# moriglia/qam-reconciliation

Hardware: AMD Instinct MI355X
Metric: decoded frames/sec @ N=64800, 50 BP iters; achieved HBM GB/s vs roofline (higher is better)
Workload: dtype f64; 1 GPU; dvbs2_4pam; code=DVB-S2-rate-1/2-profile IRA N=64800, V=64800, C=32400, E=226799, batch_per_gpu=4096, global_batch=4096, bps=2, fused_demap=False, parallelism=dp1, hip_graph=False, backend=none, arithmetic=strict (glibc exp/log restated: outputs bit-identical to the reference)

## Files before the change

### qam-reconciliation_amd/csrc/decoder.hip

```cpp
#include <atomic>
#include <functional>

#include "debug_check.hpp"
#include "glibc_math.hpp"
#include "qamr_internal.hpp"
#include "strict_pack.hpp"
#include "host_build.hpp"

namespace qr {

enum CheckMode { kFirst = 0, kNormal = 1, kParityOnly = 2 };

enum DebugSite {
    kDbgLaneFrame = 1,
    kDbgNarrowFrame = 2,
    kDbgNarrowNode = 3,
    kDbgRepackList = 4,
    kDbgRepackSlot = 5,
    kDbgRepackFid = 6,
    kDbgCompact = 7,
    kDbgResPost = 8,
    kDbgResMsg = 9,
    kDbgFewCheck = 17,
    kDbgFewPost = 18,
// ... 79 lines not shown
    double *post;
    const uint8_t *active;
    int ld, f_off;
    Geom g;
    unsigned nbx;
    const int32_t *alist, *acount;
    unsigned nby;
    int gs;
    int boost;
    int32_t *finite;
    double fin_bound;
    int fin_B;
    const int32_t *sel;
    const double *lappr_w[2];
    double *post_w;
    const double *c2v_alt;
    int transit;
};

enum RangeSelField { kSelOn = 0, kSelW = 1, kSelRepacks = 2, kSelArrive = 3, kSelBuf = 4, kSelTransit = 5, kSelInts = 6 };

__device__ __forceinline__ void select_range(CheckArgs &a) {
    if (a.sel && sld(a.sel + kSelOn)) {
        const int b = sld(a.sel + kSelBuf);
        a.post = a.post_w;
        a.synd = b ? a.synd_w[1] : a.synd_w[0];
        double *const c0 = a.c2v, *const c1 = a.c2v_alt;
        a.c2v = b ? c1 : c0;
        a.transit = sld(a.sel + kSelTransit);
        a.c2v_rd = a.transit ? (b ? c0 : c1) : a.c2v;
    }
}
__device__ __forceinline__ void select_range(VarArgs &a) {
    if (a.sel && sld(a.sel + kSelOn)) {
        const int b = sld(a.sel + kSelBuf);
        a.lappr = b ? a.lappr_w[1] : a.lappr_w[0];
        a.post = a.post_w;
        a.transit = sld(a.sel + kSelTransit);
        if (a.transit ? !b : b) a.c2v = a.c2v_alt;
    }
}

__device__ __forceinline__ bool frames_block_live(const int32_t *acount, unsigned by, int lft) {
    return !acount || (int)(by << lft) < *acount;
}
__device__ __forceinline__ int lane_frame(const int32_t *alist, const int32_t *acount, int f_off, int p, bool &live) {
    live = true;
    if (!alist) return f_off + p;
    const int cnt = *acount;
    live = p < cnt;
    const int f = alist[f_off + (live ? p : cnt - 1)];
    QR_DCHECK(f >= f_off + (live ? p : cnt - 1), kDbgLaneFrame, f, f_off + p);
    return f;
}


template <int D, int MODE, bool NT, bool TRANSIT = false>
struct CheckIn {
    double p[D], c[D];
    int base;
    uint8_t sb;
    __device__ __forceinline__ void load(const CheckArgs &a, int64_t ci, int f) {
        const int ld = a.ld;
        const uint32_t b8 = (uint32_t)f * 8u;
        const int cc = sld(a.checks + ci);
        base = sld(a.chk_ptr + cc);
        sb = *at_byte(row_ptr(a.synd, cc, ld), (uint32_t)f);
#pragma unroll
        for (int i = 0; i < D; ++i) p[i] = ld_row<false>(row_ptr(a.post, sld(a.chk_var + base + i), ld), b8, ld);
    }
    __device__ __forceinline__ void load_c(const CheckArgs &a, int fc) {
        if (MODE != kNormal) return;
        const uint32_t b8 = (uint32_t)fc * 8u;
        const double *c2v = TRANSIT ? a.c2v_rd : a.c2v;
#pragma unroll
        for (int i = 0; i < D; ++i) c[i] = ld_row<NT>(row_ptr(c2v, sld(a.chk_edge + base + i), a.ld), b8, a.ld);
    }
};

__device__ __forceinline__ uint32_t sign_mask(uint8_t sb) { return sb ? 0x80000000u : 0u; }
__device__ __forceinline__ double apply_sign(double x, uint32_t smask) { return g_make(g_hi(x) ^ smask, g_lo(x)); }

constexpr int kPackMaxDeg = 10;
constexpr int kPackLdsDoubles = 4 * kPackWaveDoubles;
template <int D>
constexpr bool kPacked = D <= kPackMaxDeg;

template <int D, bool NT, bool FIN = false>
__device__ __forceinline__ void check_exact(const CheckArgs &a, const double (&m)[D], int base, uint8_t sb, uint32_t b8,
                                            const GlibcTablesBP &tab, const GlibcK &K, double *hb = nullptr,
                                            bool live = true) {
    const int ld = a.ld;
    const double s = sb ? -1.0 : 1.0;
    if constexpr (kPacked<D>) {
        double out[D];
        double *wb = hb + (threadIdx.x >> 6) * kPackWaveDoubles;
        check_strict_packed<D, FIN ? kClampFinite : kClampFull>(m, out, wb, tab, K);
        const uint32_t smask = sign_mask(sb);
#pragma unroll
        for (int i = 0; i < D; ++i)
            if (live) st_row<NT>(row_ptr(a.c2v, sld(a.chk_edge + base + i), ld), b8, ld, apply_sign(out[i], smask));
        return;
    }
    double F[D - 1];
    F[0] = m[0];
#pragma unroll
    for (int i = 1; i < D - 1; ++i) F[i] = box_plus_strict(F[i - 1], m[i], tab, K);
    if (live) st_row<NT>(row_ptr(a.c2v, sld(a.chk_edge + base + D - 1), ld), b8, ld, s * F[D - 2]);
    double Bn = m[D - 1];
#pragma unroll
    for (int i = D - 2; i > 0; --i) {
        const double o = s * box_plus_strict(F[i - 1], Bn, tab, K);
        if (live) st_row<NT>(row_ptr(a.c2v, sld(a.chk_edge + base + i), ld), b8, ld, o);
        Bn = box_plus_strict(Bn, m[i], tab, K);
    }
    if (live) st_row<NT>(row_ptr(a.c2v, sld(a.chk_edge + base), ld), b8, ld, s * Bn);
}

template <int D, int MODE, bool NT, bool FIN = false, bool TRANSIT = false>
__device__ __forceinline__ void check_block(const CheckArgs &a, unsigned bx, unsigned by, int per,
                                            const GlibcTablesBP &tab, double *hb) {
    const int ft = 1 << a.g.lft;
    const int nsub = 256 >> a.g.lft;
    bool live;
    const int lp = (int)(by << a.g.lft) + (threadIdx.x & (ft - 1));
    const int fl = lane_frame(a.alist, a.acount, a.f_off, lp, live);
    const int f = TRANSIT ? a.f_off + lp : fl;
    const int sub = __builtin_amdgcn_readfirstlane(threadIdx.x >> a.g.lft);
    const bool act = live && a.active[f] != 0;
    if (!wave_any(act)) return;
    int64_t ci = (int64_t)bx * per * nsub + sub;
    if (ci >= a.n_checks) return;
    uint32_t bad = 0;
    const auto K = GlibcK::pinned();
    constexpr bool kPrefetch = !kPacked<D>;
    CheckIn<D, MODE, NT, TRANSIT> nx;
    nx.load(a, ci, f);
    for (int j = 0; j < per; ++j) {
        nx.load_c(a, TRANSIT ? fl : f);
        uint32_t par = nx.sb;
        double m[D];
#pragma unroll
        for (int i = 0; i < D; ++i) {
            const double p = nx.p[i];
            if (MODE != kFirst) par ^= (p < 0.0) ? 1u : 0u;
            if (MODE == kNormal) m[i] = p - nx.c[i];
            else m[i] = p;
        }
        struct { int base; uint8_t sb; } cur = {nx.base, nx.sb};
        const int64_t cn = ci + nsub;
        const bool more = (j + 1 < per) && cn < a.n_checks;
        if (kPrefetch && more) nx.load(a, cn, f);
        if (MODE != kFirst) bad |= (par == 1u) ? 1u : 0u;
        if (MODE != kParityOnly) {
            const uint32_t b8 = (uint32_t)f * 8u;
            check_exact<D, NT, FIN>(a, m, cur.base, cur.sb, b8, tab, K, hb, live);
        }
        if (!more) break;
        if (!kPrefetch) nx.load(a, cn, f);
        ci = cn;
    }
    if (MODE != kFirst && bad && act && live) a.unsat[f] = 1;
}

template <bool INIT, bool NT, bool TRANSIT = false>
__device__ __forceinline__ void var_block(const VarArgs &a, unsigned bx, unsigned by) {
    const int ft = 1 << a.g.lft;
    const int nsub = 256 >> a.g.lft;
    const int ld = a.ld;
    bool live;
    const int lp = (int)(by << a.g.lft) + (threadIdx.x & (ft - 1));
    const int fl = lane_frame(a.alist, a.acount, a.f_off, lp, live);
    const int f = TRANSIT ? a.f_off + lp : fl;
    const int fc = TRANSIT ? fl : f;
    const int sub = __builtin_amdgcn_readfirstlane(threadIdx.x >> a.g.lft);
    const bool act = a.active[f] != 0;
    if (!live || (!INIT && !act)) return;
    if (INIT && f >= a.fin_B) return;
    const int64_t v0 = (int64_t)bx * a.g.per * nsub + sub;
    bool big = false;
    for (int j = 0; j < a.g.per; ++j) {
        const int64_t v = v0 + (int64_t)j * nsub;
        if (v >= a.V) break;
        const int b = sld(a.var_ptr + v), e = sld(a.var_ptr + v + 1);
        double p = ld_msg<NT>(&a.lappr[(size_t)v * ld + f]);
        if (INIT) {
            big |= !(__builtin_fabs(p) < a.fin_bound);
            if (act && e > b) p = p + 0.0;
        } else {
            for (int k = b; k < e; ++k) p += ld_msg<NT>(&a.c2v[(size_t)sld(a.var_edge + k) * ld + fc]);
        }
        a.post[(size_t)v * ld + f] = p;
    }
    if (INIT && a.finite && big && f < a.fin_B) *a.finite = 0;
}

constexpr int kNarrowFrames = 16;
constexpr int kNarrowNodes = 256 / kNarrowFrames;
constexpr int kNarrowW = 64;

__device__ __forceinline__ bool range_narrow(const int32_t *sel, const int32_t *acount) {
    return sel && acount && sld(sel + kSelOn) && sld(sel + kSelW) <= kNarrowW && !sld(sel + kSelTransit);
}
__device__ __forceinline__ uint32_t narrow_tasks(int64_t n, const int32_t *acount, int &lg) {
    const int ngrp = (sld(acount) + kNarrowFrames - 1) / kNarrowFrames;
    lg = ngrp > 2 ? 2 : ngrp > 1 ? 1 : 0;
    return ngrp > 0 ? (uint32_t)((n + kNarrowNodes - 1) / kNarrowNodes) << lg : 0u;
}

template <int D>
__device__ __forceinline__ void check_narrow(const CheckArgs &a, uint32_t task, int lg, const GlibcTablesBP &tab,
                                             double *hb, const GlibcK &K) {
    bool live;
    const int grp = (int)(task & ((1u << lg) - 1u));
    const int f = lane_frame(a.alist, a.acount, a.f_off, grp * kNarrowFrames + (int)(threadIdx.x % kNarrowFrames), live);
    const bool act = live && a.active[f] != 0;
    if (!wave_any(act)) return;
    const int64_t ci = (int64_t)(task >> lg) * kNarrowNodes + threadIdx.x / kNarrowFrames;
    const bool valid = ci < a.n_checks;
    const int cc = a.checks[valid ? ci : a.n_checks - 1];
    int base = a.chk_ptr[cc];
    QR_DCHECK(f >= a.f_off && f < a.f_off + kNarrowW, kDbgNarrowFrame, f, a.f_off);
    QR_DCHECK(cc >= 0 && base >= 0 && a.chk_ptr[cc + 1] - base == D, kDbgNarrowNode, cc, base);
    const size_t ld = a.ld;
    const uint8_t sb = a.synd[(size_t)cc * ld + f];
    uint32_t par = sb;
    double m[D];
#pragma unroll
    for (int i = 0; i < D; ++i) {
        const double p = a.post[(size_t)a.chk_var[base + i] * ld + f];
        par ^= (p < 0.0) ? 1u : 0u;
        m[i] = p - a.c2v[(size_t)a.chk_edge[base + i] * ld + f];
    }
    double out[D];
    check_strict_packed<D, kClampFull>(m, out, hb + (threadIdx.x >> 6) * kPackWaveDoubles, tab, K);
    __asm__ volatile("" : "+v"(base));
    const double s = sb ? -1.0 : 1.0;
    if (valid && act) {
#pragma unroll
        for (int i = 0; i < D; ++i) a.c2v[(size_t)a.chk_edge[base + i] * ld + f] = s * out[i];
        if (par == 1u) a.unsat[f] = 1;
    }
}

template <int D>
__device__ __forceinline__ void check_narrow_sweep(const CheckArgs &a, GlibcTablesBP &tab, double *hb) {
    int lg;
    const uint32_t ntask = narrow_tasks(a.n_checks, a.acount, lg);
    const uint32_t nb = gridDim.x * gridDim.y, b = blockIdx.y * gridDim.x + blockIdx.x;
    if (b >= ntask) return;
    stage_glibc_tables(&tab, a.gglibc);
    const auto K = GlibcK::pinned();
    for (uint32_t t = b; t < ntask; t += nb) check_narrow<D>(a, t, lg, tab, hb, K);
}

__device__ __forceinline__ void var_narrow_sweep(const VarArgs &a) {
    int lg;
    const uint32_t ntask = narrow_tasks(a.V, a.acount, lg);
    const uint32_t nb = gridDim.x * gridDim.y;
    const size_t ld = a.ld;
    for (uint32_t t = blockIdx.y * gridDim.x + blockIdx.x; t < ntask; t += nb) {
        bool live;
        const int grp = (int)(t & ((1u << lg) - 1u));
        const int f = lane_frame(a.alist, a.acount, a.f_off, grp * kNarrowFrames + (int)(threadIdx.x % kNarrowFrames), live);
        const int64_t v = (int64_t)(t >> lg) * kNarrowNodes + threadIdx.x / kNarrowFrames;
        if (!live || v >= a.V || !a.active[f]) continue;
        QR_DCHECK(f >= a.f_off && f < a.f_off + kNarrowW, kDbgNarrowFrame, f, a.f_off);
        double p = a.lappr[(size_t)v * ld + f];
        const int b = a.var_ptr[v], e = a.var_ptr[v + 1];
        for (int k = b; k < e; ++k) p += a.c2v[(size_t)a.var_edge[k] * ld + f];
        a.post[(size_t)v * ld + f] = p;
    }
}

#if QR_EXPERIMENT_CLOCK
__device__ unsigned long long g_clk[3];
__device__ unsigned long long g_wgt[2 * kWgTimes];
#endif
template <int D, int MODE, bool NT>
__global__ void __launch_bounds__(256) __attribute__((amdgpu_waves_per_eu(1, 8))) k_check(CheckArgs a) {
    __shared__ GlibcTablesBP tab;
    __shared__ double hb[kPackLdsDoubles];
    select_range(a);
    if constexpr (MODE == kNormal && kPacked<D>) {
        if (range_narrow(a.sel, a.acount)) {
            check_narrow_sweep<D>(a, tab, hb);
            return;
        }
    }
    unsigned bx = blockIdx.x, by = blockIdx.y;
    int per = a.g.per;
    if (a.nmain) {
        if (bx < a.nmain) {
            by = 1 + bx / a.nbx;
            bx -= (by - 1) * a.nbx;
        } else {
            bx -= a.nmain;
            by = 0;
            per = a.per_t;
        }
    }
    if (!frames_block_live(a.acount, by, a.g.lft)) return;
#if QR_EXPERIMENT_CLOCK
    ClkScope clk(D == 7 && MODE == kNormal, g_clk, g_wgt);
#endif
    if (MODE != kParityOnly) stage_glibc_tables(&tab, a.gglibc);
    if constexpr (MODE == kNormal) {
        if (a.transit) {
            check_block<D, MODE, NT, false, true>(a, bx, by, per, tab, hb);
            return;
        }
    }
    if constexpr (MODE != kParityOnly && kPacked<D>) {
        if (a.finite && sld(a.finite)) {
            check_block<D, MODE, NT, true>(a, bx, by, per, tab, hb);
            return;
        }
    }
    check_block<D, MODE, NT, false>(a, bx, by, per, tab, hb);
}

template <bool INIT, bool NT, bool TRANSIT>
__device__ __forceinline__ void var_sweep_body(const VarArgs &a);

template <bool INIT, bool NT>
__global__ void __launch_bounds__(256) k_var(VarArgs a) {
    select_range(a);
    if (!INIT && range_narrow(a.sel, a.acount)) {
        var_narrow_sweep(a);
        return;
    }
    if (!INIT && a.transit) var_sweep_body<INIT, NT, true>(a);
    else var_sweep_body<INIT, NT, false>(a);
}

template <bool INIT, bool NT, bool TRANSIT>
__device__ __forceinline__ void var_sweep_body(const VarArgs &a) {
    if (a.gs) {
        unsigned ny = a.nby, stride = gridDim.x;
        if (a.boost > 1) {
            const unsigned w = gridDim.x / (unsigned)a.boost;
            unsigned live = a.nby;
            if (a.acount) live = min(a.nby, (unsigned)((*a.acount + (1 << a.g.lft) - 1) >> a.g.lft));
            const unsigned m = live ? min((unsigned)a.boost, max(1u, a.nby / live)) : 1u;
            stride = w * m;
            ny = live;
            if (blockIdx.x >= stride) return;
        }
        const unsigned n = a.nbx * ny;
        for (unsigned t = blockIdx.x; t < n; t += stride) {
            const unsigned by = t / a.nbx, bx = t - by * a.nbx;
            if (frames_block_live(a.acount, by, a.g.lft)) var_block<INIT, NT, TRANSIT>(a, bx, by);
        }
        return;
    }
    if (!frames_block_live(a.acount, blockIdx.y, a.g.lft)) return;
    var_block<INIT, NT, TRANSIT>(a, blockIdx.x, blockIdx.y);
}


struct IterArgs {
    const int32_t *checks;
    int64_t n_checks;
    const int32_t *chk_ptr, *chk_edge, *chk_var, *var_ptr, *var_edge;
    const double *lappr;
    double *post;
    const double *c2v_in;
    double *c2v_out;
    const uint8_t *synd;
    uint8_t *active, *success;
    int32_t *iters;
    const uint8_t *unsat_s;
    uint8_t *unsat_p;
    int32_t status_iter;
    int ld, f_off;
    Geom g;
    unsigned nbx;
    const GlibcTables *gglibc;
    const int32_t *finite;
};

template <int D, bool FIN>
__device__ __forceinline__ void iter_block(const IterArgs &a, unsigned bx, unsigned by, const GlibcTablesBP &tab,
                                           double *hb) {
    const int ft = 1 << a.g.lft;
    const int nsub = 256 >> a.g.lft;
    const int ld = a.ld;
    const int f = a.f_off + (int)(by << a.g.lft) + (threadIdx.x & (ft - 1));
    const int sub = __builtin_amdgcn_readfirstlane(threadIdx.x >> a.g.lft);
    const bool was = a.active[f] != 0;
    const bool act = was && (!a.unsat_s || a.unsat_s[f] != 0);
    int64_t ci = (int64_t)bx * a.g.per * nsub + sub;
    if (ci == 0 && was && !act) {
        a.success[f] = 1;
        a.iters[f] = a.status_iter;
        a.active[f] = 0;
    }
    if (!wave_any(act)) return;
    const auto K = GlibcK::pinned();
    const uint32_t b8 = (uint32_t)f * 8u;
    uint32_t bad = 0;
    for (int j = 0; j < a.g.per; ++j, ci += nsub) {
        if (ci >= a.n_checks) break;
        const int cc = sld(a.checks + ci);
        const int base = sld(a.chk_ptr + cc);
        uint32_t par = *at_byte(row_ptr(a.synd, cc, ld), (uint32_t)f);
        double m[D];
#pragma unroll
        for (int i = 0; i < D; ++i) {
            const int v = sld(a.chk_var + base + i), e = sld(a.chk_edge + base + i);
            const int vb = sld(a.var_ptr + v), ve = sld(a.var_ptr + v + 1);
            double p = ld_row<false>(row_ptr(a.lappr, v, ld), b8, ld);
            double own = 0.0;
            for (int k = vb; k < ve; ++k) {
                const int ek = sld(a.var_edge + k);
                const double c = a.c2v_in ? ld_row<false>(row_ptr(a.c2v_in, ek, ld), b8, ld) : 0.0;
                p += c;
                own = (ek == e) ? c : own;
            }
            if (act && sld(a.var_edge + vb) == e) st_row<false>(row_ptr(a.post, v, ld), b8, ld, p);
            par ^= (p < 0.0) ? 1u : 0u;
            m[i] = p - own;
        }
        bad |= (par == 1u) ? 1u : 0u;
        if (a.c2v_out) {
            const double s = *at_byte(row_ptr(a.synd, cc, ld), (uint32_t)f) ? -1.0 : 1.0;
            double out[D];
            double *wb = hb + (threadIdx.x >> 6) * kPackWaveDoubles;
            check_strict_packed<D, FIN ? kClampFinite : kClampFull>(m, out, wb, tab, K);
#pragma unroll
            for (int i = 0; i < D; ++i)
                if (act) st_row<false>(row_ptr(a.c2v_out, sld(a.chk_edge + base + i), ld), b8, ld, s * out[i]);
        }
    }
    if (a.unsat_p && bad && act) a.unsat_p[f] = 1;
}

template <int D>
__global__ void __launch_bounds__(256) __attribute__((amdgpu_waves_per_eu(1, 8))) k_iter(IterArgs a) {
    __shared__ GlibcTablesBP tab;
    __shared__ double hb[4 * kPackWaveDoubles];
    if (a.c2v_out) stage_glibc_tables(&tab, a.gglibc);
    if (a.finite && sld(a.finite)) iter_block<D, true>(a, blockIdx.x, blockIdx.y, tab, hb);
    else iter_block<D, false>(a, blockIdx.x, blockIdx.y, tab, hb);
}

constexpr int kResThreads = 512;
constexpr int kResMaxIter = 10000;
constexpr int kResStaticLds = (int)sizeof(GlibcTablesBP) + (kResThreads / 64) * kPackWaveDoubles * 8;

struct ResArgs {
    int C, V, B, ld, max_it;
    const int32_t *chk_var;
    const int32_t *var_ptr, *var_msg;
    const double *lappr;
    const uint8_t *synd;
    double *post;
    uint8_t *success;
    int32_t *iters;
    const GlibcTables *gglibc;
    double fin_bound;
    int dv;
    int32_t *rsel;
    int w0, w1;
};

template <int D>
__device__ __forceinline__ uint32_t res_parity(const ResArgs &a, int f, const double *post) {
    uint32_t bad = 0;
    for (int c = threadIdx.x; c < a.C; c += kResThreads) {
        uint32_t par = a.synd[(size_t)c * a.ld + f];
#pragma unroll
        for (int i = 0; i < D; ++i) par ^= (post[a.chk_var[c * D + i]] < 0.0) ? 1u : 0u;
        bad |= (par == 1u) ? 1u : 0u;
    }
    return bad;
}

__device__ __forceinline__ void res_finish(const ResArgs &a, int f, const double *post, int ok, int32_t it) {
    for (int v = threadIdx.x; v < a.V; v += kResThreads) a.post[(size_t)v * a.ld + f] = post[v];
    if (threadIdx.x == 0) {
        a.success[f] = (uint8_t)ok;
        a.iters[f] = it;
    }
}

template <int D, bool FIN>
__device__ __forceinline__ void resident_loop(const ResArgs &a, int f, double *msg, double *post,
                                              const GlibcTablesBP &tab, double *wb) {
    const int tid = threadIdx.x;
    const size_t ld = a.ld;
    const auto K = GlibcK::pinned();
    const int c_first = min(tid, a.C - 1);
    const uint8_t sb_first = a.synd[(size_t)c_first * ld + f];
    const bool lreg = a.V <= 2 * kResThreads;
    const double l0 = lreg && tid < a.V ? a.lappr[(size_t)tid * ld + f] : 0.0;
    const double l1 = lreg && tid + kResThreads < a.V ? a.lappr[(size_t)(tid + kResThreads) * ld + f] : 0.0;
    const int dv = lreg ? a.dv : 0;
    uint32_t vm[3] = {0u, 0u, 0u};
#pragma unroll
    for (int q = 0; q < 3; ++q) {
        if (q < dv) {
            const uint32_t i0 = tid < a.V ? (uint32_t)a.var_msg[tid * dv + q] : 0u;
            const uint32_t i1 = tid + kResThreads < a.V ? (uint32_t)a.var_msg[(tid + kResThreads) * dv + q] : 0u;
            vm[q] = i0 | i1 << 16;
        }
    }
    for (int t = 1; t <= a.max_it; ++t) {
        uint32_t bad = 0;
        for (int c0 = 0; c0 < a.C; c0 += kResThreads) {
            if (c0 + (tid & ~63) >= a.C) break;
            const int c = c0 + tid;
            const bool live = c < a.C;
            const int cc = live ? c : a.C - 1;
            const uint8_t sb = c0 == 0 ? sb_first : a.synd[(size_t)cc * ld + f];
            uint32_t par = sb;
            double m[D];
#pragma unroll
            for (int i = 0; i < D; ++i) {
                QR_DCHECK(a.chk_var[cc * D + i] >= 0 && a.chk_var[cc * D + i] < a.V, kDbgResPost, cc, a.chk_var[cc * D + i]);
                QR_DCHECK(i * a.C + cc < a.C * D, kDbgResMsg, cc, i);
                const double p = post[a.chk_var[cc * D + i]];
                par ^= (p < 0.0) ? 1u : 0u;
                m[i] = p - msg[i * a.C + cc];
            }
            if (live) bad |= (par == 1u) ? 1u : 0u;
            double out[D];
            check_strict_packed<D, FIN ? kClampFinite : kClampFull>(m, out, wb, tab, K);
            const uint32_t smask = sign_mask(sb);
            if (live) {
#pragma unroll
                for (int i = 0; i < D; ++i) msg[i * a.C + cc] = apply_sign(out[i], smask);
            }
        }
        const int any_bad = __syncthreads_or((int)bad);
        if (t >= 2 && !any_bad) {
            res_finish(a, f, post, 1, t - 1);
            return;
        }
        if (dv) {
            double p0 = l0, p1 = l1;
#pragma unroll
            for (int q = 0; q < 3; ++q) {
                if (q < dv) {
                    QR_DCHECK((vm[q] & 0xFFFFu) < (uint32_t)(a.C * D) && (vm[q] >> 16) < (uint32_t)(a.C * D), kDbgResMsg,
                              vm[q] & 0xFFFFu, vm[q] >> 16);
                    const double m0 = msg[vm[q] & 0xFFFFu], m1 = msg[vm[q] >> 16];
                    p0 += m0;
                    p1 += m1;
                }
            }
            if (tid < a.V) post[tid] = p0;
            if (tid + kResThreads < a.V) post[tid + kResThreads] = p1;
        }
        for (int v0 = dv ? a.V : tid; v0 < a.V; v0 += 2 * kResThreads) {
            const int v1 = v0 + kResThreads;
            const bool two = v1 < a.V;
            const int w1 = two ? v1 : v0;
            double p0 = lreg ? l0 : a.lappr[(size_t)v0 * ld + f];
            double p1 = lreg ? l1 : a.lappr[(size_t)w1 * ld + f];
            const int b0 = a.var_ptr[v0], e0 = a.var_ptr[v0 + 1];
            const int b1 = a.var_ptr[w1], e1 = a.var_ptr[w1 + 1];
            const int n = max(e0 - b0, e1 - b1);
            for (int q = 0; q < n; ++q) {
                const bool h0 = b0 + q < e0, h1 = b1 + q < e1;
                QR_DCHECK(a.var_msg[h0 ? b0 + q : 0] < a.C * D && a.var_msg[h1 ? b1 + q : 0] < a.C * D, kDbgResMsg,
                          a.var_msg[h0 ? b0 + q : 0], a.var_msg[h1 ? b1 + q : 0]);
                const double m0 = msg[a.var_msg[h0 ? b0 + q : 0]];
                const double m1 = msg[a.var_msg[h1 ? b1 + q : 0]];
                if (h0) p0 += m0;
                if (h1) p1 += m1;
            }
            post[v0] = p0;
            if (two) post[v1] = p1;
        }
        __syncthreads();
    }
    const int any_bad = __syncthreads_or((int)res_parity<D>(a, f, post));
    res_finish(a, f, post, any_bad ? 0 : 1, a.max_it);
}

template <int D>
__global__ void __launch_bounds__(kResThreads) __attribute__((amdgpu_waves_per_eu(4, 8))) k_resident(ResArgs a) {
    extern __shared__ double res_dyn[];
    __shared__ GlibcTablesBP tab;
    __shared__ double hb[(kResThreads / 64) * kPackWaveDoubles];
#if QR_EXPERIMENT_CLOCK
    ClkScope clk(true, g_clk, nullptr);
#endif
    const int q = (a.B + 7) / 8;
    const int f = (int)(blockIdx.x & 7u) * q + (int)(blockIdx.x >> 3);
    if (blockIdx.x == 0 && threadIdx.x < 2 * kSelInts)
        a.rsel[threadIdx.x] = (threadIdx.x % kSelInts == kSelW) ? (threadIdx.x < kSelInts ? a.w0 : a.w1) : 0;
    if (f >= a.B) return;
    stage_glibc_tables(&tab, a.gglibc);
    const int tid = threadIdx.x;
    const size_t ld = a.ld;
    double *msg = res_dyn, *post = res_dyn + (size_t)a.C * D;
    for (int s = tid; s < a.C * D; s += kResThreads) msg[s] = 0.0;
    bool small = true;
    for (int v = tid; v < a.V; v += kResThreads) {
        const double x = a.lappr[(size_t)v * ld + f];
        small &= __builtin_fabs(x) < a.fin_bound;
        post[v] = (a.var_ptr[v + 1] > a.var_ptr[v]) ? x + 0.0 : x;
    }
    const int fin = __syncthreads_and((int)small);
    if (!__syncthreads_or((int)res_parity<D>(a, f, post))) {
        for (int v = tid; v < a.V; v += kResThreads) a.post[(size_t)v * ld + f] = a.lappr[(size_t)v * ld + f];
        if (tid == 0) {
            a.success[f] = 1;
            a.iters[f] = 0;
        }
        return;
    }
    double *wb = hb + (tid >> 6) * kPackWaveDoubles;
    if (fin) resident_loop<D, true>(a, f, msg, post, tab, wb);
    else resident_loop<D, false>(a, f, msg, post, tab, wb);
}

constexpr int kFewThreads = 256;

struct FewCheckArgs {
    const int32_t *checks;
    int n;
    int64_t base;
    int64_t E, V, C;
    const int32_t *chk_ptr, *chk_var;
    const double *post;
    double *msg;
    const uint8_t *synd;
    const uint8_t *active;
    uint8_t *unsat;
    const int32_t *finite;
    const GlibcTables *gglibc;
};

template <int D, bool FIN, class ST>
__device__ __forceinline__ void few_update(const double (&m)[D], uint32_t smask, double *wb, const GlibcTablesBP &tab,
                                           const GlibcK &K, ST store) {
    if constexpr (kPacked<D>) {
        double out[D];
        check_strict_packed<D, FIN ? kClampFinite : kClampFull>(m, out, wb, tab, K);
#pragma unroll
        for (int i = 0; i < D; ++i) store(i, apply_sign(out[i], smask));
    } else {
        double F[D - 1];
        F[0] = m[0];
#pragma unroll
        for (int i = 1; i < D - 1; ++i) F[i] = box_plus_strict(F[i - 1], m[i], tab, K);
        store(D - 1, apply_sign(F[D - 2], smask));
        double Bn = m[D - 1];
#pragma unroll
        for (int i = D - 2; i > 0; --i) {
            store(i, apply_sign(box_plus_strict(F[i - 1], Bn, tab, K), smask));
            Bn = box_plus_strict(Bn, m[i], tab, K);
        }
        store(0, apply_sign(Bn, smask));
    }
}

template <int D, int MODE, bool FIN>
__device__ __forceinline__ void few_check_body(const FewCheckArgs &a, int f, const GlibcTablesBP &tab, double *hb) {
    const int j0 = (int)(blockIdx.x * kFewThreads + threadIdx.x);
    if ((j0 & ~63) >= a.n) return;
    const bool live = j0 < a.n;
    const int j = live ? j0 : a.n - 1;
    const int cc = a.checks[j];
    QR_DCHECK(cc >= 0 && cc < a.C && a.chk_ptr[cc + 1] - a.chk_ptr[cc] == D, kDbgFewCheck, cc, j);
    const int cb = a.chk_ptr[cc];
    const double *post = a.post + (size_t)f * a.V;
    double *msg = a.msg + (size_t)f * a.E + a.base + j;
    const uint8_t sb = a.synd[(size_t)f * a.C + cc];
    uint32_t par = sb;
    double m[D];
#pragma unroll
    for (int i = 0; i < D; ++i) {
        const int v = a.chk_var[cb + i];
        QR_DCHECK(v >= 0 && v < a.V, kDbgFewPost, cc, v);
        QR_DCHECK(a.base + (int64_t)i * a.n + j >= 0 && a.base + (int64_t)i * a.n + j < a.E, kDbgFewSlot, cc, i);
        const double p = post[v];
        if (MODE != kFirst) par ^= (p < 0.0) ? 1u : 0u;
        if (MODE == kNormal) m[i] = p - msg[(size_t)i * a.n];
        else m[i] = p;
    }
    if (MODE != kFirst && live && par == 1u) a.unsat[f] = 1;
    if constexpr (MODE != kParityOnly) {
        const auto K = GlibcK::pinned();
        few_update<D, FIN>(m, sign_mask(sb), hb + (threadIdx.x >> 6) * kPackWaveDoubles, tab, K, [&](int i, double x) {
            if (live) msg[(size_t)i * a.n] = x;
        });
    }
}

template <int D, int MODE>
__global__ void __launch_bounds__(kFewThreads) k_few_check(FewCheckArgs a) {
    __shared__ GlibcTablesBP tab;
    __shared__ double hb[(kFewThreads / 64) * kPackWaveDoubles];
    const int f = (int)blockIdx.y;
    if (!a.active[f]) return;
    if (MODE != kParityOnly) stage_glibc_tables(&tab, a.gglibc);
    if constexpr (MODE != kParityOnly && kPacked<D>) {
        if (sld(a.finite)) {
            few_check_body<D, MODE, true>(a, f, tab, hb);
            return;
        }
    }
    few_check_body<D, MODE, false>(a, f, tab, hb);
}

struct FewVarArgs {
    int64_t V, E;
    const int32_t *var_ptr, *var_slot;
    const double *lappr;
    const double *msg;
    double *post;
    const uint8_t *active;
    int32_t *finite;
    double fin_bound;
};

template <bool INIT>
__global__ void __launch_bounds__(kFewThreads) k_few_var(FewVarArgs a) {
    const int f = (int)blockIdx.y;
    const bool act = a.active[f] != 0;
    if (!INIT && !act) return;
    const int64_t v = (int64_t)blockIdx.x * kFewThreads + threadIdx.x;
    if (v >= a.V) return;
    const int b = a.var_ptr[v], e = a.var_ptr[v + 1];
    double p = a.lappr[(size_t)f * a.V + v];
    if (INIT) {
        if (a.finite && !(__builtin_fabs(p) < a.fin_bound)) *a.finite = 0;
        if (act && e > b) p = p + 0.0;
    } else {
        const double *msg = a.msg + (size_t)f * a.E;
        for (int k = b; k < e; ++k) {
            QR_DCHECK(a.var_slot[k] >= 0 && a.var_slot[k] < a.E, kDbgFewSlot, v, a.var_slot[k]);
            p += msg[a.var_slot[k]];
        }
    }
    a.post[(size_t)f * a.V + v] = p;
}

constexpr int kMaxTemplDeg = 16;

template <int MODE>
__global__ void __launch_bounds__(256) k_check_generic(CheckArgs a) {
    __shared__ GlibcTablesBP tab;
    select_range(a);
    if (MODE != kParityOnly) stage_glibc_tables(&tab, a.gglibc);
    const int ft = 1 << a.g.lft;
    const int nsub = 256 >> a.g.lft;
    const int ld = a.ld;
    if (!frames_block_live(a.acount, blockIdx.y, a.g.lft)) return;
    bool live;
    const int f = lane_frame(a.alist, a.acount, a.f_off, (int)(blockIdx.y << a.g.lft) + (threadIdx.x & (ft - 1)), live);
    const int sub = __builtin_amdgcn_readfirstlane(threadIdx.x >> a.g.lft);
    if (!live || !a.active[f]) return;
    const auto K = GlibcK::pinned();
    const int64_t c0 = (int64_t)blockIdx.x * a.g.per * nsub + sub;
    const uint32_t b8 = (uint32_t)f * 8u;
    uint32_t bad = 0;
    for (int j = 0; j < a.g.per; ++j) {
        const int64_t ci = c0 + (int64_t)j * nsub;
        if (ci >= a.n_checks) break;
        const int c = sld(a.checks + ci);
        const int base = sld(a.chk_ptr + c);
        const int d = sld(a.chk_ptr + c + 1) - base;
        const uint8_t sb = *at_byte(row_ptr(a.synd, c, ld), (uint32_t)f);
        const double s = sb ? -1.0 : 1.0;
        uint32_t par = sb;
        auto msg = [&](int i, bool count) {
            const double p = *at_byte(row_ptr(a.post, sld(a.chk_var + base + i), ld), b8);
            if (count && MODE != kFirst) par ^= (p < 0.0) ? 1u : 0u;
            return (MODE == kNormal) ? p - *at_byte(row_ptr(a.c2v, sld(a.chk_edge + base + i), ld), b8) : p;
        };
        if (MODE == kParityOnly) {
            for (int i = 0; i < d; ++i) (void)msg(i, true);
            bad |= (par == 1u) ? 1u : 0u;
            continue;
        }
// ... 1484 lines not shown
```

### qam-reconciliation_amd/csrc/strict_pack.hpp

```cpp
#pragma once
#include "glibc_math.hpp"

namespace qr {

typedef __attribute__((address_space(3))) double lds_f64;

constexpr int kPackMaxJobs = 8;
constexpr int kPackWaveDoubles = 64 * kPackMaxJobs + 64;

__host__ __device__ constexpr int pack_out_round(int D, int i) {
    return ((i - 1) > (D - 2 - i) ? (i - 1) : (D - 2 - i)) + 1;
}

enum { kClampNone = 0, kClampFull = 1, kClampFinite = 2 };
template <int CL = kClampFull, class TT = GlibcTables>
__device__ __forceinline__ void h_packed(const double *t, double *h, int nj, double *wb, const TT &T,
                                         const GlibcK &K) {
    constexpr int S = kPackWaveDoubles;
    const uint32_t lane = __lane_id();
    uint32_t addr[kPackMaxJobs];
    uint32_t nN = 0;
    const uint32_t wb0 = (uint32_t)(uintptr_t)(lds_f64 *)wb / 8u;
#pragma unroll
    for (int j = 0; j < kPackMaxJobs; ++j) {
        if (j >= nj) break;
        double xe;
        if constexpr (CL == kClampFull) xe = -fabs(g_make((fabs(t[j]) > 37.5) ? 0x4042C000u : g_hi(t[j]), g_lo(t[j])));
        else if constexpr (CL == kClampFinite) xe = __builtin_fmax(-fabs(t[j]), -700.0);
        else xe = -fabs(t[j]);
        const double u = 1.0 + g_exp_neg(xe, T, K);
        const bool near = g_hi(u) < 0x3FF10900u;
        const uint64_t mk = __ballot(near);
        const uint32_t x = near ? wb0 : wb0 + (uint32_t)(S - 1) - lane - 64u * (uint32_t)j;
        const uint32_t a = __builtin_amdgcn_mbcnt_hi((uint32_t)(mk >> 32), __builtin_amdgcn_mbcnt_lo((uint32_t)mk, x));
        addr[j] = (a + nN) << 3;
        *(lds_f64 *)(uintptr_t)addr[j] = u;
        nN += (uint32_t)__popcll(mk);
    }
    const uint32_t nT = 64u * (uint32_t)nj - nN;
    __builtin_amdgcn_fence(__ATOMIC_RELEASE, "wavefront");
    __builtin_amdgcn_fence(__ATOMIC_ACQUIRE, "wavefront");
    double *wn = wb + lane;
    double *wt = wb + (S - 1 - 64 * kPackMaxJobs) - lane;
    double cur = wn[0];
#pragma unroll
    for (int q = 0; q <= kPackMaxJobs; ++q) {
        if (64u * (uint32_t)q >= nN) break;
        const double nxt = (q < kPackMaxJobs) ? wn[64 * (q + 1)] : 0.0;
        wn[64 * q] = g_log_near1(cur, K);
        cur = nxt;
    }
    cur = wt[64 * kPackMaxJobs];
#pragma unroll
    for (int q = 0; q <= kPackMaxJobs; ++q) {
        if (64u * (uint32_t)q >= nT) break;
        const double nxt = (q < kPackMaxJobs) ? wt[64 * (kPackMaxJobs - q - 1)] : 0.0;
        wt[64 * (kPackMaxJobs - q)] = g_log_table(cur, g_hi(cur), T, K);
        cur = nxt;
    }
    __builtin_amdgcn_fence(__ATOMIC_RELEASE, "wavefront");
    __builtin_amdgcn_fence(__ATOMIC_ACQUIRE, "wavefront");
#pragma unroll
    for (int j = 0; j < kPackMaxJobs; ++j) {
        if (j >= nj) break;
        h[j] = *(const lds_f64 *)(uintptr_t)addr[j];
    }
    __builtin_amdgcn_fence(__ATOMIC_RELEASE, "wavefront");
    __builtin_amdgcn_fence(__ATOMIC_ACQUIRE, "wavefront");
}

__device__ __forceinline__ double signed_min_packed(double a, double b) {
    const double mn = __builtin_fmin(__builtin_fabs(a), __builtin_fabs(b));
    return g_make(g_bfi(0x7FFFFFFFu, g_hi(mn), g_hi(a) ^ g_hi(b)), g_lo(mn));
}

template <int D, int CL = kClampFull, class TT = GlibcTables>
__device__ __forceinline__ void check_strict_packed(const double (&m)[D], double (&out)[D], double *wb, const TT &T,
                                                    const GlibcK &K) {
    if constexpr (D == 2) {
        out[0] = m[1];
        out[1] = m[0];
    } else {
        double F[D], Bv[D];
        F[0] = m[0];
        Bv[D - 1] = m[D - 1];
#pragma unroll
        for (int r = 1; r <= D - 2; ++r) {
            int kind[4], idx[4];
            int k = 0;
            kind[k] = 0, idx[k] = r, ++k;
            kind[k] = 1, idx[k] = D - 1 - r, ++k;
#pragma unroll
            for (int i = 1; i <= D - 2; ++i)
                if (pack_out_round(D, i) == r) kind[k] = 2, idx[k] = i, ++k;
            double t[8], h[8], sm[4];
#pragma unroll
            for (int q = 0; q < 4; ++q) {
                if (q >= k) break;
                const double a = kind[q] == 0 ? F[r - 1] : kind[q] == 1 ? Bv[D - r] : F[idx[q] - 1];
                const double b = kind[q] == 0 ? m[r] : kind[q] == 1 ? m[D - 1 - r] : Bv[idx[q] + 1];
                sm[q] = signed_min_packed(a, b);
                t[2 * q] = a + b;
                t[2 * q + 1] = a - b;
            }
            h_packed<CL>(t, h, 2 * k, wb, T, K);
#pragma unroll
            for (int q = 0; q < 4; ++q) {
                if (q >= k) break;
                const double v = (sm[q] + h[2 * q]) - h[2 * q + 1];
                if (kind[q] == 0) F[idx[q]] = v;
                else if (kind[q] == 1) Bv[idx[q]] = v;
                else out[idx[q]] = v;
            }
        }
        out[0] = Bv[1];
        out[D - 1] = F[D - 2];
    }
}

}
```

Before: 9892 frames/s.

## Pipeline packed box-plus rounds across consecutive degree-7 checks in first sweep

Adds a software-pipelined check sweep for degree-7 checks in the first (kFirst) mode. The final rounds of one check's packed box-plus forward/backward computation are merged with the early rounds of the next check, so each wave-wide h_packed call handles more jobs, and the next check's early inputs are loaded ahead of time. The per-wave LDS scratch grows to 12 jobs, but only for this path, and those kernels get a 60-VGPR cap. The aim is fewer per-round LDS/log calls and fences, and better latency hiding. The cost is more LDS and register pressure, plus added template complexity.

Measured after the change: 9895 frames/s (median of 5 runs). Within noise of the previous version (+0.0%).

```diff
diff --git a/qam-reconciliation_amd/csrc/decoder.hip b/qam-reconciliation_amd/csrc/decoder.hip
--- a/qam-reconciliation_amd/csrc/decoder.hip
+++ b/qam-reconciliation_amd/csrc/decoder.hip
@@ -185,11 +185,14 @@
 __device__ __forceinline__ double apply_sign(double x, uint32_t smask) { return g_make(g_hi(x) ^ smask, g_lo(x)); }
 
 constexpr int kPackMaxDeg = 10;
-constexpr int kPackLdsDoubles = 4 * kPackWaveDoubles;
 template <int D>
 constexpr bool kPacked = D <= kPackMaxDeg;
-
-template <int D, bool NT, bool FIN = false>
+template <int D, int MODE>
+constexpr bool kPipelined = D == 7 && MODE == kFirst;
+template <int D, int MODE>
+constexpr int kCheckWaveDoubles = kPipelined<D, MODE> ? kPackWaveDoubles : kPackRoundDoubles;
+
+template <int D, bool NT, bool FIN = false, int MODE = kNormal>
 __device__ __forceinline__ void check_exact(const CheckArgs &a, const double (&m)[D], int base, uint8_t sb, uint32_t b8,
                                             const GlibcTablesBP &tab, const GlibcK &K, double *hb = nullptr,
                                             bool live = true) {
@@ -197,7 +200,7 @@
     const double s = sb ? -1.0 : 1.0;
     if constexpr (kPacked<D>) {
         double out[D];
-        double *wb = hb + (threadIdx.x >> 6) * kPackWaveDoubles;
+        double *wb = hb + (threadIdx.x >> 6) * kCheckWaveDoubles<D, MODE>;
         check_strict_packed<D, FIN ? kClampFinite : kClampFull>(m, out, wb, tab, K);
         const uint32_t smask = sign_mask(sb);
 #pragma unroll
@@ -220,9 +223,73 @@
     if (live) st_row<NT>(row_ptr(a.c2v, sld(a.chk_edge + base), ld), b8, ld, s * Bn);
 }
 
+template <int D, int MODE, bool NT, bool FIN>
+__device__ __forceinline__ void check_block_pipe(const CheckArgs &a, unsigned bx, unsigned by, int per,
+                                                 const GlibcTablesBP &tab, double *hb) {
+    static_assert(kPipelined<D, MODE> && MODE != kParityOnly && pack_depth(D) >= 1, "a pipelined packed degree");
+    const int ft = 1 << a.g.lft;
+    const int nsub = 256 >> a.g.lft;
+    const int ld = a.ld;
+    bool live;
+    const int lp = (int)(by << a.g.lft) + (threadIdx.x & (ft - 1));
+    const int f = lane_frame(a.alist, a.acount, a.f_off, lp, live);
+    const int sub = __builtin_amdgcn_readfirstlane(threadIdx.x >> a.g.lft);
+    const bool act = live && a.active[f] != 0;
+    if (!wave_any(act)) return;
+    int64_t ci = (int64_t)bx * per * nsub + sub;
+    if (ci >= a.n_checks) return;
+    uint32_t bad = 0;
+    const auto K = GlibcK::pinned();
+    const uint32_t b8 = (uint32_t)f * 8u;
+    PackOpsWave<FIN ? kClampFinite : kClampFull, GlibcTablesBP> ops{hb + (threadIdx.x >> 6) * kPackWaveDoubles, tab, K};
+    struct Edge {
+        int base;
+        uint32_t smask;
+    } ec, en;
+    int j = 0;
+    auto more = [&]() { return (j + 1 < per) && ci + nsub < a.n_checks; };
+    uint32_t par = 0;
+    auto take = [&](PackCheck<D> &s, auto part) {
+        constexpr int P = decltype(part)::value;
+        Edge &e = P ? en : ec;
+        if constexpr (P != 2) {
+            const int cc = sld(a.checks + (P ? ci + nsub : ci));
+            e.base = sld(a.chk_ptr + cc);
+            const uint8_t sb = *at_byte(row_ptr(a.synd, cc, ld), (uint32_t)f);
+            e.smask = sign_mask(sb);
+            par = sb;
+        }
+#pragma unroll
+        for (int i = 0; i < D; ++i) {
+            if (P && pack_input_early(D, pack_depth(D), i) != (P == 1)) continue;
+            const double p = ld_row<false>(row_ptr(a.post, sld(a.chk_var + e.base + i), ld), b8, ld);
+            if (MODE != kFirst) par ^= (p < 0.0) ? 1u : 0u;
+            if (MODE == kNormal) s.m[i] = p - ld_row<NT>(row_ptr(a.c2v, sld(a.chk_edge + e.base + i), ld), b8, ld);
+            else s.m[i] = p;
+        }
+        if (P != 1 && MODE != kFirst) bad |= (par == 1u) ? 1u : 0u;
+    };
+    auto put = [&](auto rc, const PackCheck<D> &s) {
+        pack_round_outputs<D, decltype(rc)::value>(s, [&](int i, double v) {
+            if (live) st_row<NT>(row_ptr(a.c2v, sld(a.chk_edge + ec.base + i), ld), b8, ld, apply_sign(v, ec.smask));
+        });
+    };
+    auto advance = [&]() {
+        ec = en;
+        ci += nsub;
+        ++j;
+    };
+    pack_walk<D, pack_depth(D)>(ops, more, take, put, advance);
+    if (MODE != kFirst && bad && act && live) a.unsat[f] = 1;
+}
+
 template <int D, int MODE, bool NT, bool FIN = false, bool TRANSIT = false>
 __device__ __forceinline__ void check_block(const CheckArgs &a, unsigned bx, unsigned by, int per,
                                             const GlibcTablesBP &tab, double *hb) {
+    if constexpr (kPipelined<D, MODE> && !TRANSIT) {
+        check_block_pipe<D, MODE, NT, FIN>(a, bx, by, per, tab, hb);
+        return;
+    }
     const int ft = 1 << a.g.lft;
     const int nsub = 256 >> a.g.lft;
     bool live;
@@ -257,7 +324,7 @@
         if (MODE != kFirst) bad |= (par == 1u) ? 1u : 0u;
         if (MODE != kParityOnly) {
             const uint32_t b8 = (uint32_t)f * 8u;
-            check_exact<D, NT, FIN>(a, m, cur.base, cur.sb, b8, tab, K, hb, live);
+            check_exact<D, NT, FIN, MODE>(a, m, cur.base, cur.sb, b8, tab, K, hb, live);
         }
         if (!more) break;
         if (!kPrefetch) nx.load(a, cn, f);
@@ -336,7 +403,7 @@
         m[i] = p - a.c2v[(size_t)a.chk_edge[base + i] * ld + f];
     }
     double out[D];
-    check_strict_packed<D, kClampFull>(m, out, hb + (threadIdx.x >> 6) * kPackWaveDoubles, tab, K);
+    check_strict_packed<D, kClampFull>(m, out, hb + (threadIdx.x >> 6) * kCheckWaveDoubles<D, kNormal>, tab, K);
     __asm__ volatile("" : "+v"(base));
     const double s = sb ? -1.0 : 1.0;
     if (valid && act) {
@@ -381,9 +448,7 @@
 __device__ unsigned long long g_wgt[2 * kWgTimes];
 #endif
 template <int D, int MODE, bool NT>
-__global__ void __launch_bounds__(256) __attribute__((amdgpu_waves_per_eu(1, 8))) k_check(CheckArgs a) {
-    __shared__ GlibcTablesBP tab;
-    __shared__ double hb[kPackLdsDoubles];
+__device__ __forceinline__ void check_sweep(CheckArgs &a, GlibcTablesBP &tab, double *hb) {
     select_range(a);
     if constexpr (MODE == kNormal && kPacked<D>) {
         if (range_narrow(a.sel, a.acount)) {
@@ -422,6 +487,24 @@
     }
     check_block<D, MODE, NT, false>(a, bx, by, per, tab, hb);
 }
+
+template <int D, int MODE, bool NT>
+__global__ void __launch_bounds__(256) __attribute__((amdgpu_waves_per_eu(1, 8))) k_check(CheckArgs a) {
+    __shared__ GlibcTablesBP tab;
+    __shared__ double hb[4 * kCheckWaveDoubles<D, MODE>];
+    check_sweep<D, MODE, NT>(a, tab, hb);
+}
+#define QR_CHECK_CAPPED(NT)                                                                                           \
+    template <>                                                                                                       \
+    __global__ void __launch_bounds__(256) __attribute__((amdgpu_num_vgpr(60))) k_check<7, kFirst, NT>(CheckArgs a) { \
+        __shared__ GlibcTablesBP tab;                                                                                 \
+        __shared__ double hb[4 * kCheckWaveDoubles<7, kFirst>];                                                       \
+        check_sweep<7, kFirst, NT>(a, tab, hb);                                                                       \
+    }
+static_assert(kPipelined<7, kFirst>, "the capped kernels are the pipelined sweep's");
+QR_CHECK_CAPPED(false)
+QR_CHECK_CAPPED(true)
+#undef QR_CHECK_CAPPED
 
 template <bool INIT, bool NT, bool TRANSIT>
 __device__ __forceinline__ void var_sweep_body(const VarArgs &a);
@@ -529,7 +612,7 @@
         if (a.c2v_out) {
             const double s = *at_byte(row_ptr(a.synd, cc, ld), (uint32_t)f) ? -1.0 : 1.0;
             double out[D];
-            double *wb = hb + (threadIdx.x >> 6) * kPackWaveDoubles;
+            double *wb = hb + (threadIdx.x >> 6) * kPackRoundDoubles;
             check_strict_packed<D, FIN ? kClampFinite : kClampFull>(m, out, wb, tab, K);
 #pragma unroll
             for (int i = 0; i < D; ++i)
@@ -542,7 +625,7 @@
 template <int D>
 __global__ void __launch_bounds__(256) __attribute__((amdgpu_waves_per_eu(1, 8))) k_iter(IterArgs a) {
     __shared__ GlibcTablesBP tab;
-    __shared__ double hb[4 * kPackWaveDoubles];
+    __shared__ double hb[4 * kPackRoundDoubles];
     if (a.c2v_out) stage_glibc_tables(&tab, a.gglibc);
     if (a.finite && sld(a.finite)) iter_block<D, true>(a, blockIdx.x, blockIdx.y, tab, hb);
     else iter_block<D, false>(a, blockIdx.x, blockIdx.y, tab, hb);
@@ -550,7 +633,7 @@
 
 constexpr int kResThreads = 512;
 constexpr int kResMaxIter = 10000;
-constexpr int kResStaticLds = (int)sizeof(GlibcTablesBP) + (kResThreads / 64) * kPackWaveDoubles * 8;
+constexpr int kResStaticLds = (int)sizeof(GlibcTablesBP) + (kResThreads / 64) * kPackRoundDoubles * 8;
 
 struct ResArgs {
     int C, V, B, ld, max_it;
@@ -687,7 +770,7 @@
 __global__ void __launch_bounds__(kResThreads) __attribute__((amdgpu_waves_per_eu(4, 8))) k_resident(ResArgs a) {
     extern __shared__ double res_dyn[];
     __shared__ GlibcTablesBP tab;
-    __shared__ double hb[(kResThreads / 64) * kPackWaveDoubles];
+    __shared__ double hb[(kResThreads / 64) * kPackRoundDoubles];
 #if QR_EXPERIMENT_CLOCK
     ClkScope clk(true, g_clk, nullptr);
 #endif
@@ -716,7 +799,7 @@
         }
         return;
     }
-    double *wb = hb + (tid >> 6) * kPackWaveDoubles;
+    double *wb = hb + (tid >> 6) * kPackRoundDoubles;
     if (fin) resident_loop<D, true>(a, f, msg, post, tab, wb);
     else resident_loop<D, false>(a, f, msg, post, tab, wb);
 }
@@ -789,7 +872,7 @@
     if (MODE != kFirst && live && par == 1u) a.unsat[f] = 1;
     if constexpr (MODE != kParityOnly) {
         const auto K = GlibcK::pinned();
-        few_update<D, FIN>(m, sign_mask(sb), hb + (threadIdx.x >> 6) * kPackWaveDoubles, tab, K, [&](int i, double x) {
+        few_update<D, FIN>(m, sign_mask(sb), hb + (threadIdx.x >> 6) * kPackRoundDoubles, tab, K, [&](int i, double x) {
             if (live) msg[(size_t)i * a.n] = x;
         });
     }
@@ -798,7 +881,7 @@
 template <int D, int MODE>
 __global__ void __launch_bounds__(kFewThreads) k_few_check(FewCheckArgs a) {
     __shared__ GlibcTablesBP tab;
-    __shared__ double hb[(kFewThreads / 64) * kPackWaveDoubles];
+    __shared__ double hb[(kFewThreads / 64) * kPackRoundDoubles];
     const int f = (int)blockIdx.y;
     if (!a.active[f]) return;
     if (MODE != kParityOnly) stage_glibc_tables(&tab, a.gglibc);
diff --git a/qam-reconciliation_amd/csrc/strict_pack.hpp b/qam-reconciliation_amd/csrc/strict_pack.hpp
--- a/qam-reconciliation_amd/csrc/strict_pack.hpp
+++ b/qam-reconciliation_amd/csrc/strict_pack.hpp
@@ -1,28 +1,33 @@
 #pragma once
+#include <utility>
+
 #include "glibc_math.hpp"
 
 namespace qr {
 
 typedef __attribute__((address_space(3))) double lds_f64;
 
-constexpr int kPackMaxJobs = 8;
-constexpr int kPackWaveDoubles = 64 * kPackMaxJobs + 64;
+constexpr int kPackRoundJobs = 8;
+constexpr int kPackMaxJobs = 12;
+__host__ __device__ constexpr int pack_wave_doubles(int mj) { return 64 * mj + 64; }
+constexpr int kPackRoundDoubles = pack_wave_doubles(kPackRoundJobs);
+constexpr int kPackWaveDoubles = pack_wave_doubles(kPackMaxJobs);
 
 __host__ __device__ constexpr int pack_out_round(int D, int i) {
     return ((i - 1) > (D - 2 - i) ? (i - 1) : (D - 2 - i)) + 1;
 }
 
 enum { kClampNone = 0, kClampFull = 1, kClampFinite = 2 };
-template <int CL = kClampFull, class TT = GlibcTables>
+template <int CL = kClampFull, int MJ = kPackRoundJobs, class TT = GlibcTables>
 __device__ __forceinline__ void h_packed(const double *t, double *h, int nj, double *wb, const TT &T,
                                          const GlibcK &K) {
-    constexpr int S = kPackWaveDoubles;
+    constexpr int S = pack_wave_doubles(MJ);
     const uint32_t lane = __lane_id();
-    uint32_t addr[kPackMaxJobs];
+    uint32_t addr[MJ];
     uint32_t nN = 0;
     const uint32_t wb0 = (uint32_t)(uintptr_t)(lds_f64 *)wb / 8u;
 #pragma unroll
-    for (int j = 0; j < kPackMaxJobs; ++j) {
+    for (int j = 0; j < MJ; ++j) {
         if (j >= nj) break;
         double xe;
         if constexpr (CL == kClampFull) xe = -fabs(g_make((fabs(t[j]) > 37.5) ? 0x4042C000u : g_hi(t[j]), g_lo(t[j])));
@@ -41,27 +46,27 @@
     __builtin_amdgcn_fence(__ATOMIC_RELEASE, "wavefront");
     __builtin_amdgcn_fence(__ATOMIC_ACQUIRE, "wavefront");
     double *wn = wb + lane;
-    double *wt = wb + (S - 1 - 64 * kPackMaxJobs) - lane;
+    double *wt = wb + (S - 1 - 64 * MJ) - lane;
     double cur = wn[0];
 #pragma unroll
-    for (int q = 0; q <= kPackMaxJobs; ++q) {
+    for (int q = 0; q <= MJ; ++q) {
         if (64u * (uint32_t)q >= nN) break;
-        const double nxt = (q < kPackMaxJobs) ? wn[64 * (q + 1)] : 0.0;
+        const double nxt = (q < MJ) ? wn[64 * (q + 1)] : 0.0;
         wn[64 * q] = g_log_near1(cur, K);
         cur = nxt;
     }
-    cur = wt[64 * kPackMaxJobs];
-#pragma unroll
-    for (int q = 0; q <= kPackMaxJobs; ++q) {
+    cur = wt[64 * MJ];
+#pragma unroll
+    for (int q = 0; q <= MJ; ++q) {
         if (64u * (uint32_t)q >= nT) break;
-        const double nxt = (q < kPackMaxJobs) ? wt[64 * (kPackMaxJobs - q - 1)] : 0.0;
-        wt[64 * (kPackMaxJobs - q)] = g_log_table(cur, g_hi(cur), T, K);
+        const double nxt = (q < MJ) ? wt[64 * (MJ - q - 1)] : 0.0;
+        wt[64 * (MJ - q)] = g_log_table(cur, g_hi(cur), T, K);
         cur = nxt;
     }
     __builtin_amdgcn_fence(__ATOMIC_RELEASE, "wavefront");
     __builtin_amdgcn_fence(__ATOMIC_ACQUIRE, "wavefront");
 #pragma unroll
-    for (int j = 0; j < kPackMaxJobs; ++j) {
+    for (int j = 0; j < MJ; ++j) {
         if (j >= nj) break;
         h[j] = *(const lds_f64 *)(uintptr_t)addr[j];
     }
@@ -103,7 +108,7 @@
                 t[2 * q] = a + b;
                 t[2 * q + 1] = a - b;
             }
-            h_packed<CL>(t, h, 2 * k, wb, T, K);
+            h_packed<CL, kPackRoundJobs>(t, h, 2 * k, wb, T, K);
 #pragma unroll
             for (int q = 0; q < 4; ++q) {
                 if (q >= k) break;
@@ -118,4 +123,189 @@
     }
 }
 
-}
+
+enum { kBpF = 0, kBpB = 1, kBpO = 2 };
+enum { kRefM = 0, kRefF = 1, kRefB = 2 };
+struct PackRef {
+    int arr, i;
+};
+struct PackBp {
+    int kind, idx;
+    PackRef a, b;
+};
+
+__host__ __device__ constexpr int pack_rounds(int D) { return D > 2 ? D - 2 : 0; }
+__host__ __device__ constexpr int pack_round_count(int D, int r) {
+    int k = 2;
+    for (int i = 1; i <= D - 2; ++i)
+        if (pack_out_round(D, i) == r) ++k;
+    return k;
+}
+__host__ __device__ constexpr PackBp pack_round_bp(int D, int r, int q) {
+    if (q == 0) return {kBpF, r, {kRefF, r - 1}, {kRefM, r}};
+    if (q == 1) return {kBpB, D - 1 - r, {kRefB, D - r}, {kRefM, D - 1 - r}};
+    int k = 2;
+    for (int i = 1; i <= D - 2; ++i)
+        if (pack_out_round(D, i) == r) {
+            if (k == q) return {kBpO, i, {kRefF, i - 1}, {kRefB, i + 1}};
+            ++k;
+        }
+    return {-1, 0, {0, 0}, {0, 0}};
+}
+#ifndef QR_PACK_DEPTH
+#define QR_PACK_DEPTH 1
+#endif
+__host__ __device__ constexpr int pack_depth(int D, int dmax = QR_PACK_DEPTH) {
+    const int d = pack_rounds(D) / 2;
+    return d < dmax ? d : dmax;
+}
+__host__ __device__ constexpr int pack_own_calls(int D, int d) { return pack_rounds(D) - d; }
+__host__ __device__ constexpr int pack_call_round(int D, int d, int k) { return d + 1 + k; }
+__host__ __device__ constexpr int pack_call_next(int D, int d, int k) {
+    const int rc = d + 1 + k, R = pack_rounds(D);
+    return rc > R - d ? rc - (R - d) : 0;
+}
+struct PackCall {
+    int j, rc, rn;
+};
+__host__ __device__ constexpr int pack_walk_calls(int D, int n, int d) {
+    return (n > 0 && pack_rounds(D) > 0) ? d + n * pack_own_calls(D, d) : 0;
+}
+__host__ __device__ constexpr PackCall pack_walk_call(int D, int n, int d, int c) {
+    if (c < d) return {-1, 0, c + 1};
+    const int own = pack_own_calls(D, d), j = (c - d) / own, k = (c - d) % own;
+    return {j, pack_call_round(D, d, k), j + 1 < n ? pack_call_next(D, d, k) : 0};
+}
+
+template <int D>
+struct PackCheck {
+    double m[D], F[D], B[D], out[D];
+    __host__ __device__ __forceinline__ void start() {
+        F[0] = m[0];
+        B[D - 1] = m[D - 1];
+        if constexpr (D == 2) out[0] = m[1], out[1] = m[0];
+    }
+};
+
+template <int ARR, int I, int D>
+__host__ __device__ __forceinline__ double pack_ref(const PackCheck<D> &s) {
+    static_assert(I >= 0 && I < D, "operand index");
+    if constexpr (ARR == kRefM) return s.m[I];
+    else if constexpr (ARR == kRefF) return s.F[I];
+    else return s.B[I];
+}
+template <int D, int R, int O, int Q, class OPS>
+__host__ __device__ __forceinline__ void pack_bp_in(const PackCheck<D> &s, double *t, double *sm, OPS &ops) {
+    constexpr PackBp bp = pack_round_bp(D, R, Q);
+    static_assert(bp.kind >= 0, "box-plus index");
+    const double a = pack_ref<bp.a.arr, bp.a.i>(s), b = pack_ref<bp.b.arr, bp.b.i>(s);
+    sm[O + Q] = ops.signed_min(a, b);
+    t[2 * (O + Q)] = a + b;
+    t[2 * (O + Q) + 1] = a - b;
+}
+template <int D, int R, int O, int Q>
+__host__ __device__ __forceinline__ void pack_bp_out(PackCheck<D> &s, const double *h, const double *sm) {
+    constexpr PackBp bp = pack_round_bp(D, R, Q);
+    const double v = (sm[O + Q] + h[2 * (O + Q)]) - h[2 * (O + Q) + 1];
+    if constexpr (bp.kind == kBpF) {
+        s.F[bp.idx] = v;
+        if constexpr (bp.idx == D - 2) s.out[D - 1] = v;
+    } else if constexpr (bp.kind == kBpB) {
+        s.B[bp.idx] = v;
+        if constexpr (bp.idx == 1) s.out[0] = v;
+    } else {
+        s.out[bp.idx] = v;
+    }
+}
+template <int D, int R, int O, class OPS, int... Q>
+__host__ __device__ __forceinline__ void pack_round_in(const PackCheck<D> &s, double *t, double *sm, OPS &ops,
+                                                       std::integer_sequence<int, Q...>) {
+    (pack_bp_in<D, R, O, Q>(s, t, sm, ops), ...);
+}
+template <int D, int R, int O, int... Q>
+__host__ __device__ __forceinline__ void pack_round_out(PackCheck<D> &s, const double *h, const double *sm,
+                                                        std::integer_sequence<int, Q...>) {
+    (pack_bp_out<D, R, O, Q>(s, h, sm), ...);
+}
+template <int D, int RC, int RN, class OPS>
+__host__ __device__ __forceinline__ void pack_call(PackCheck<D> &c, PackCheck<D> &n, OPS &ops) {
+    constexpr int kc = RC ? pack_round_count(D, RC) : 0, kn = RN ? pack_round_count(D, RN) : 0;
+    static_assert(kc + kn > 0 && 2 * (kc + kn) <= kPackMaxJobs, "arguments of one call");
+    double t[2 * (kc + kn)], h[2 * (kc + kn)], sm[kc + kn];
+    pack_round_in<D, RC, 0>(c, t, sm, ops, std::make_integer_sequence<int, kc>());
+    pack_round_in<D, RN, kc>(n, t, sm, ops, std::make_integer_sequence<int, kn>());
+    ops.template h<2 * (kc + kn)>(t, h);
+    pack_round_out<D, RC, 0>(c, h, sm, std::make_integer_sequence<int, kc>());
+    pack_round_out<D, RN, kc>(n, h, sm, std::make_integer_sequence<int, kn>());
+}
+
+template <class F, int... I>
+__host__ __device__ __forceinline__ void static_for_seq(F &&f, std::integer_sequence<int, I...>) {
+    (f(std::integral_constant<int, I>()), ...);
+}
+template <int N, class F>
+__host__ __device__ __forceinline__ void static_for(F &&f) {
+    static_for_seq(f, std::make_integer_sequence<int, N>());
+}
+
+template <int D, int RC, class F>
+__host__ __device__ __forceinline__ void pack_round_outputs(const PackCheck<D> &s, F &&f) {
+    static_for<(D > 2 ? D - 2 : 0)>([&](auto i1) {
+        constexpr int i = decltype(i1)::value + 1;
+        if constexpr (pack_out_round(D, i) == RC) f(i, s.out[i]);
+    });
+    if constexpr (RC == D - 2) f(0, s.out[0]), f(D - 1, s.out[D - 1]);
+}
+
+__host__ __device__ constexpr bool pack_input_early(int D, int d, int i) { return i <= d || i >= D - 1 - d; }
+template <int D, int PD, class OPS, class MORE, class TAKE, class PUT, class ADV>
+__host__ __device__ __forceinline__ void pack_walk(OPS &ops, MORE &&more, TAKE &&take, PUT &&put, ADV &&advance) {
+    constexpr int d = PD, own = pack_own_calls(D, d);
+    static_assert(d >= 0 && 2 * d <= pack_rounds(D), "early and late rounds must not meet");
+    PackCheck<D> cur, nxt;
+    take(cur, std::integral_constant<int, 0>());
+    cur.start();
+    static_for<d>([&](auto r) { pack_call<D, 0, decltype(r)::value + 1>(cur, cur, ops); });
+    for (;;) {
+        const bool m = more();
+        if constexpr (pack_rounds(D) == 0) put(std::integral_constant<int, 0>(), cur);
+        static_for<own - d>([&](auto k) {
+            constexpr int rc = pack_call_round(D, d, decltype(k)::value);
+            pack_call<D, rc, 0>(cur, cur, ops);
+            put(std::integral_constant<int, rc>(), cur);
+        });
+        if (!m) {
+            static_for<d>([&](auto k) {
+                constexpr int rc = pack_call_round(D, d, own - d + decltype(k)::value);
+                pack_call<D, rc, 0>(cur, cur, ops);
+                put(std::integral_constant<int, rc>(), cur);
+            });
+            break;
+        }
+        take(nxt, std::integral_constant<int, 1>());
+        nxt.start();
+        static_for<d>([&](auto k) {
+            constexpr int kk = own - d + decltype(k)::value;
+            constexpr int rc = pack_call_round(D, d, kk);
+            pack_call<D, rc, pack_call_next(D, d, kk)>(cur, nxt, ops);
+            put(std::integral_constant<int, rc>(), cur);
+        });
+        take(nxt, std::integral_constant<int, 2>());
+        cur = nxt;
+        advance();
+    }
+}
+
+template <int CL, class TT>
+struct PackOpsWave {
+    double *wb;
+    const TT &T;
+    const GlibcK &K;
+    __device__ __forceinline__ double signed_min(double a, double b) const { return signed_min_packed(a, b); }
+    template <int NJ>
+    __device__ __forceinline__ void h(const double *t, double *h) const {
+        h_packed<CL, kPackMaxJobs>(t, h, NJ, wb, T, K);
+    }
+};
+
+}
```
